# marqo-ai/marqo

Measured on NVIDIA H100. Metric: embeddings/s (open_clip/ViT-L-14 image vectorise, batch 256 per GPU), higher is better.
Workload: dtype bf16

## Files before the change

### marqo_b200/csrc/gemm.cu

```cuda
#include "gemm.cuh"

#include <mutex>
#include <type_traits>

#include "ptx.cuh"

namespace mb {
namespace gemm {

constexpr int BM = 128;
constexpr int BN = 128;
constexpr int BK = 64;
constexpr int WG_K = 16;
constexpr int STAGES = 3;
constexpr int MMA_THREADS = 256;
constexpr uint32_t A_STAGE_BYTES = BM * BK * 2;
constexpr uint32_t B_STAGE_BYTES = BN * BK * 2;
constexpr uint32_t STAGE_BYTES = A_STAGE_BYTES + B_STAGE_BYTES;
constexpr uint32_t BARRIER_BYTES = 256;
constexpr size_t SMEM_BYTES = (size_t)STAGES * STAGE_BYTES + 1024  + BARRIER_BYTES + 2 * BN * 4 ;
constexpr int EPI_ROWS = BM / 2;
constexpr uint32_t EPI_BOX_BYTES = EPI_ROWS * 128;
static_assert(4 * EPI_BOX_BYTES == STAGE_BYTES, "a warpgroup's fp32 64 x 128 block is one ring stage");

constexpr int P_BN = 256;
constexpr int P_STAGES = 3;
constexpr uint32_t P_STAGE_BYTES = A_STAGE_BYTES + P_BN * BK * 2;
constexpr uint32_t P_RING_BYTES = P_STAGES * P_STAGE_BYTES;
constexpr uint32_t EPI_BYTES = 4 * EPI_BOX_BYTES;
constexpr int PERSISTENT_THREADS = 128 + MMA_THREADS;
constexpr size_t P_SMEM_BYTES = 1024  + P_RING_BYTES + 2 * EPI_BYTES + 2 * P_BN * 4 + BARRIER_BYTES;
static_assert(P_SMEM_BYTES <= 227 * 1024, "over the opt-in shared memory of an H100 CTA");
static_assert(P_BN * 2 * EPI_ROWS == EPI_BYTES, "a warpgroup's bf16 64 x 256 block is one epilogue buffer");

enum Producer { PROD_TMA = 0, PROD_PATCH = 1, PROD_CONV = 2 };

template <bool GATHER>
constexpr int threads() { return MMA_THREADS + (GATHER ? 128 : 32); }

struct Params {
    int M, N, K;
    int tiles_m, tiles_n;
    Epilogue ep;
    const uint8_t* img;
    int g;
    int patch;
    int row_bytes;
    int seg;
    int kbpd;
    float nscale[3], nshift[3];
    int cls;
};

__device__ __forceinline__ float ex2_approx(float x) {
    float y;
    asm("ex2.approx.ftz.f32 %0, %1;" : "=f"(y) : "f"(x));
    return y;
}

__device__ __forceinline__ float gelu_erf(float x) {
    const float a = x * 0.70710678118654752440f;
    const float t = fabsf(a);
    const float s = a * a;
    float r = fmaf(-2.49374837e-5f, t, 5.52836593e-4f);
    const float u = fmaf(-5.60337594e-3f, t, 3.49920232e-2f);
    r = fmaf(r, s, u);
    r = fmaf(r, t, -1.54047912e-1f);
    r = fmaf(r, t, -9.15890168e-1f);
    r = fmaf(r, t, -1.85700115e-1f);
    r = fmaf(r, t, -1.44269504f * t);
    const float e = copysignf(1.0f - ex2_approx(r), a);
    const float hx = 0.5f * x;
    return fmaf(hx, e, hx);
}

__device__ __forceinline__ __half2 gelu_erf_h2(__half2 x) {
    const __half2 a = __hmul2(x, __float2half2_rn(0.70710678118654752440f));
    const __half2 t = __habs2(a);
    const __half2 s = __hmul2(a, a);
    __half2 r = __hfma2(__float2half2_rn(-2.49374837e-5f), t, __float2half2_rn(5.52836593e-4f));
    const __half2 u = __hfma2(__float2half2_rn(-5.60337594e-3f), t, __float2half2_rn(3.49920232e-2f));
    r = __hfma2(r, s, u);
    r = __hfma2(r, t, __float2half2_rn(-1.54047912e-1f));
    r = __hfma2(r, t, __float2half2_rn(-9.15890168e-1f));
    r = __hfma2(r, t, __float2half2_rn(-1.85700115e-1f));
    r = __hfma2(r, t, __hmul2(t, __float2half2_rn(-1.44269504f)));
    const __half2 e = h2exp2(r);
    const __half2 om = __hsub2(__float2half2_rn(1.0f), e);
    const uint32_t eb = (*reinterpret_cast<const uint32_t*>(&om) & 0x7fff7fffu) | (*reinterpret_cast<const uint32_t*>(&a) & 0x80008000u);
    const __half2 erfv = *reinterpret_cast<const __half2*>(&eb);
    const __half2 hx = __hmul2(x, __float2half2_rn(0.5f));
    return __hfma2(hx, erfv, hx);
}

__device__ __forceinline__ float quick_gelu(float x) {
    return x / (1.0f + ex2_approx(-1.702f * 1.44269504f * x));
}

__device__ __forceinline__ uint32_t sw128_offset(int row, int unit) {
    return (uint32_t)row * 128u + (uint32_t)((unit ^ (row & 7)) << 4);
}

template <int ELEM>
__device__ __forceinline__ uint32_t epi_offset(int row, int col) {
    constexpr int BOX_COLS = 128 / ELEM;
    const int byte = (col % BOX_COLS) * ELEM;
    return (uint32_t)(col / BOX_COLS) * EPI_BOX_BYTES + sw128_offset(row, byte >> 4) + (uint32_t)(byte & 15);
}

__device__ __forceinline__ void warpgroup_sync(int wg) {
    if (wg == 0)
        ptx::bar_sync<1, 128>();
    else
        ptx::bar_sync<2, 128>();
}

template <bool OUT_FP32, int ACT>
__device__ __forceinline__ float2 act(float x0, float x1) {
    if constexpr (ACT == ACT_GELU && !OUT_FP32) {
        float2 y = __half22float2(gelu_erf_h2(__floats2half2_rn(x0, x1)));
        y.x = x0 >= 65504.f ? x0 : x0 <= -65504.f ? -0.f : y.x;
        y.y = x1 >= 65504.f ? x1 : x1 <= -65504.f ? -0.f : y.y;
        return y;
    } else if constexpr (ACT == ACT_GELU)
        return make_float2(gelu_erf(x0), gelu_erf(x1));
    else if constexpr (ACT == ACT_QUICKGELU)
        return make_float2(quick_gelu(x0), quick_gelu(x1));
    else if constexpr (ACT == ACT_RELU)
        return make_float2(fmaxf(x0, 0.f), fmaxf(x1, 0.f));
    else
        return make_float2(x0, x1);
}

template <bool OUT_FP32, int ACT, int COLS>
__device__ __forceinline__ void epilogue_to_smem(const float* acc, uint32_t bias_s, uint32_t buf_s, bool residual,
                                                 int rbase, int lane) {
    static_assert(!(OUT_FP32 && ACT == ACT_RELU), "ACT_RELU writes bf16");
#pragma unroll
    for (int i = 0; i < COLS / 8; ++i) {
        const int col = 8 * i + 2 * (lane & 3);
        const float2 bv = ptx::ld_shared_f32x2(bias_s + 4 * col);
#pragma unroll
        for (int h = 0; h < 2; ++h) {
            const int r = rbase + 8 * h;
            if constexpr (ACT == ACT_RELU) {
                const uint32_t dst = buf_s + epi_offset<2>(r, col);
                float x0 = acc[4 * i + 2 * h] + bv.x, x1 = acc[4 * i + 2 * h + 1] + bv.y;
                if (residual) {
                    const uint32_t rv = ptx::ld_shared_u32(dst);
                    const float2 f = __bfloat1622float2(*reinterpret_cast<const __nv_bfloat162*>(&rv));
                    x0 += f.x;
                    x1 += f.y;
                }
                const float2 y = act<false, ACT_RELU>(x0, x1);
                ptx::st_shared_u32(dst, pack_bf16x2(y.x, y.y));
                continue;
            }
            float2 y = act<OUT_FP32, ACT>(acc[4 * i + 2 * h] + bv.x, acc[4 * i + 2 * h + 1] + bv.y);
            if constexpr (OUT_FP32) {
                const uint32_t dst = buf_s + epi_offset<4>(r, col);
                if (residual) {
                    const float2 rv = ptx::ld_shared_f32x2(dst);
                    y.x += rv.x;
                    y.y += rv.y;
                }
                ptx::st_shared_f32x2(dst, y.x, y.y);
            } else {
                ptx::st_shared_u32(buf_s + epi_offset<2>(r, col), pack_bf16x2(y.x, y.y));
            }
        }
    }
}

__device__ __forceinline__ void load_residual_boxes(const CUtensorMap* tmap_r, uint64_t* bar, uint8_t* buf, int row0,
                                                    int c0, int M, int N) {
    const int boxes = row0 < M && c0 < N ? min(4, (N - c0) / 32) : 0;
    ptx::mbar_arrive_expect_tx(bar, (uint32_t)boxes * EPI_BOX_BYTES);
    for (int b = 0; b < boxes; ++b)
        ptx::tma_load_2d(buf + b * EPI_BOX_BYTES, tmap_r, bar, c0 + 32 * b, row0, ptx::kEvictNormal);
}

__device__ __forceinline__ void load_residual_boxes_bf16(const CUtensorMap* tmap_r, uint64_t* bar, uint8_t* buf,
                                                         int row0, int c0, int M, int N) {
    const int boxes = row0 < M && c0 < N ? min(2, (N - c0 + 63) / 64) : 0;
    ptx::mbar_arrive_expect_tx(bar, (uint32_t)boxes * EPI_BOX_BYTES);
    for (int b = 0; b < boxes; ++b)
        ptx::tma_load_2d(buf + b * EPI_BOX_BYTES, tmap_r, bar, c0 + 64 * b, row0, ptx::kEvictNormal);
}

template <bool OUT_FP32, int COLS>
__device__ __forceinline__ void store_output_boxes(const CUtensorMap* tmap_o, const uint8_t* buf, int row0, int c0,
                                                   int M, int N) {
    constexpr int BOX_COLS = OUT_FP32 ? 32 : 64;
    if (row0 >= M) return;
    for (int b = 0; b * BOX_COLS < COLS && c0 + b * BOX_COLS < N; ++b)
        ptx::tma_store_2d(tmap_o, buf + b * EPI_BOX_BYTES, c0 + b * BOX_COLS, row0);
    ptx::tma_store_commit();
}

template <int PROD, bool OUT_FP32, int ACT>
__global__ void __launch_bounds__(threads<PROD != PROD_TMA>(), PROD != PROD_TMA ? 1 : 2)
gemm_kernel(const __grid_constant__ CUtensorMap tmap_a, const __grid_constant__ CUtensorMap tmap_b,
            const __grid_constant__ CUtensorMap tmap_r, const __grid_constant__ CUtensorMap tmap_o,
            const __grid_constant__ Params p) {
    constexpr bool GATHER = PROD != PROD_TMA;
    extern __shared__ uint8_t smem_raw[];
    uint8_t* smem = reinterpret_cast<uint8_t*>((reinterpret_cast<uintptr_t>(smem_raw) + 1023) & ~uintptr_t(1023));
    uint64_t* full = reinterpret_cast<uint64_t*>(smem + (size_t)STAGES * STAGE_BYTES);
    uint64_t* empty = full + STAGES;
    float* bias_s = reinterpret_cast<float*>(smem + (size_t)STAGES * STAGE_BYTES + BARRIER_BYTES);

    const int warp = __shfl_sync(0xffffffffu, threadIdx.x >> 5, 0);
    const int lane = threadIdx.x & 31;
    const int tile_m = blockIdx.x / p.tiles_n, tile_n = blockIdx.x % p.tiles_n;
    const int m0 = tile_m * BM, n0 = tile_n * BN;
    const int kblocks = p.K / BK;

    if (threadIdx.x == MMA_THREADS) {
        ptx::prefetch_tmap(&tmap_b);
        if (!GATHER) ptx::prefetch_tmap(&tmap_a);
        ptx::prefetch_tmap(&tmap_o);
        if (p.ep.residual) ptx::prefetch_tmap(&tmap_r);
        for (int i = 0; i < STAGES; ++i) {
            ptx::mbar_init(&full[i], GATHER ? 1 + 128 : 1);
            ptx::mbar_init(&empty[i], MMA_THREADS / 32);
        }
        ptx::fence_barrier_init();
    }
    __syncthreads();

    if (threadIdx.x >= MMA_THREADS) {
        const int pt = threadIdx.x - MMA_THREADS;
        if (!GATHER && pt >= 32) return;
        const uint8_t* prow = nullptr;
        const __nv_bfloat16* cimg = nullptr;
        int cy = 0, cx = 0;
        const int cH = p.g, cW = p.patch, lg_cin = p.kbpd;
        if (PROD == PROD_CONV) {
            const int r = m0 + pt;
            if (r < p.M) {
                const int hw = cH * cW;
                const int b = r / hw, rem = r - b * hw;
                cy = rem / cW;
                cx = rem - cy * cW;
                cimg = reinterpret_cast<const __nv_bfloat16*>(p.img) + ((size_t)b * hw << lg_cin);
            }
        }
        if (PROD == PROD_PATCH) {
            const int r = m0 + pt;
            const int tokens = p.g * p.g + p.cls;
            const int b = r / tokens, t = r - b * tokens - p.cls;
            if (r < p.M && t >= 0) {
                const int py = t / p.g, px = t - py * p.g;
                prow = p.img + ((size_t)b * p.g * p.patch + (size_t)py * p.patch) * p.row_bytes + (size_t)px * p.patch * 3;
            }
        }
        for (int kb = 0; kb < kblocks; ++kb) {
            const int stage = kb % STAGES;
            const uint32_t phase = (uint32_t)(kb / STAGES) & 1u;
            uint8_t* sa = smem + (size_t)stage * STAGE_BYTES;
            uint8_t* sb = sa + A_STAGE_BYTES;
            ptx::mbar_wait(&empty[stage], phase ^ 1);
            if (pt == 0) {
                ptx::mbar_arrive_expect_tx(&full[stage], GATHER ? B_STAGE_BYTES : STAGE_BYTES);
                if (!GATHER) ptx::tma_load_2d(sa, &tmap_a, &full[stage], kb * BK, m0, ptx::kEvictNormal);
                ptx::tma_load_2d(sb, &tmap_b, &full[stage], kb * BK, n0, ptx::kEvictLast);
            }
            if (PROD == PROD_CONV) {
                uint4 v[8];
#pragma unroll
                for (int u = 0; u < 8; ++u) {
                    const int k = kb * 64 + u * 8;
                    const int tap = k >> lg_cin, c = k & ((1 << lg_cin) - 1);
                    const int iy = cy + tap / 3 - 1, ix = cx + tap % 3 - 1;
                    v[u] = make_uint4(0u, 0u, 0u, 0u);
                    if (cimg != nullptr && tap < 9 && (unsigned)iy < (unsigned)cH && (unsigned)ix < (unsigned)cW)
                        v[u] = __ldg(reinterpret_cast<const uint4*>(cimg + (((size_t)iy * cW + ix) << lg_cin) + c));
                }
#pragma unroll
                for (int u = 0; u < 8; ++u) *reinterpret_cast<uint4*>(sa + sw128_offset(pt, u)) = v[u];
                ptx::fence_proxy_async_smem();
                ptx::mbar_arrive(&full[stage]);
            } else if (GATHER) {
                const int dy = kb / p.kbpd, j0 = (kb - dy * p.kbpd) * 64;
                const uint8_t* src = prow ? prow + (size_t)dy * p.row_bytes + j0 : nullptr;
                int c = j0 % 3;
#pragma unroll 1
                for (int u = 0; u < 8; ++u) {
                    uint32_t w[4];
#pragma unroll
                    for (int e = 0; e < 4; ++e) {
                        float v[2];
#pragma unroll
                        for (int h = 0; h < 2; ++h) {
                            const int j = u * 8 + e * 2 + h;
                            v[h] = (src != nullptr && j0 + j < p.seg) ? fmaf((float)__ldg(src + j), p.nscale[c], p.nshift[c]) : 0.f;
                            c = c == 2 ? 0 : c + 1;
                        }
                        w[e] = pack_bf16x2(v[0], v[1]);
                    }
                    *reinterpret_cast<uint4*>(sa + sw128_offset(pt, u)) = make_uint4(w[0], w[1], w[2], w[3]);
                }
                ptx::fence_proxy_async_smem();
                ptx::mbar_arrive(&full[stage]);
            }
        }
        for (int wg = 0; wg < 2; ++wg) {
            const int kb = kblocks + wg;
            const int stage = kb % STAGES;
            uint8_t* s = smem + (size_t)stage * STAGE_BYTES;
            ptx::mbar_wait(&empty[stage], ((uint32_t)(kb / STAGES) & 1u) ^ 1);
            if (pt == 0) {
                if (p.ep.residual != nullptr) {
                    if constexpr (ACT == ACT_RELU)
                        load_residual_boxes_bf16(&tmap_r, &full[stage], s, m0 + EPI_ROWS * wg, n0, p.M, p.N);
                    else
                        load_residual_boxes(&tmap_r, &full[stage], s, m0 + EPI_ROWS * wg, n0, p.M, p.N);
                } else
                    ptx::mbar_arrive(&full[stage]);
            }
            if (GATHER) ptx::mbar_arrive(&full[stage]);
        }
        return;
    }

    const int wg = warp >> 2;
    const Epilogue& ep = p.ep;
    float bias_t = 0.f;
    if (ep.bias != nullptr && n0 + (int)(threadIdx.x & 127) < p.N) bias_t = __ldg(ep.bias + n0 + (threadIdx.x & 127));
    float acc[BN / 2];
#pragma unroll
    for (int i = 0; i < BN / 2; ++i) acc[i] = 0.f;
    for (int kb = 0; kb < kblocks; ++kb) {
        const int stage = kb % STAGES;
        ptx::mbar_wait(&full[stage], (uint32_t)(kb / STAGES) & 1u);
        const uint32_t a_base = ptx::smem_u32(smem + (size_t)stage * STAGE_BYTES) + wg * (64 * 128);
        const uint32_t b_base = ptx::smem_u32(smem + (size_t)stage * STAGE_BYTES + A_STAGE_BYTES);
        ptx::wgmma_fence();
#pragma unroll
        for (int k = 0; k < BK / WG_K; ++k)
            ptx::wgmma_m64n128k16_bf16(acc, ptx::make_desc_k_sw128(a_base + k * WG_K * 2),
                                       ptx::make_desc_k_sw128(b_base + k * WG_K * 2), (kb | k) != 0 ? 1u : 0u);
        ptx::wgmma_commit();
        ptx::wgmma_wait<1>();
        if (kb > 0 && lane == 0) ptx::mbar_arrive(&empty[(kb - 1) % STAGES]);
    }
    ptx::wgmma_wait<0>();

    const int t = threadIdx.x & 127;
    float* wbias = bias_s + wg * BN;
    wbias[t] = bias_t;
    const int kb = kblocks + wg;
    ptx::mbar_wait(&full[kb % STAGES], (uint32_t)(kb / STAGES) & 1u);
    uint8_t* tile = smem + (size_t)(kb % STAGES) * STAGE_BYTES;
    warpgroup_sync(wg);
    const int rbase = (warp & 3) * 16 + (lane >> 2);
    epilogue_to_smem<OUT_FP32, ACT, BN>(acc, ptx::smem_u32(wbias), ptx::smem_u32(tile), ep.residual != nullptr, rbase,
                                        lane);
    ptx::fence_proxy_async_smem();
    warpgroup_sync(wg);
    if (t == 0) {
        store_output_boxes<OUT_FP32, BN>(&tmap_o, tile, m0 + EPI_ROWS * wg, n0, p.M, p.N);
        ptx::tma_store_wait_read<0>();
    }
}

template <bool OUT_FP32, int ACT>
__global__ void __launch_bounds__(PERSISTENT_THREADS, 1)
gemm_persistent_kernel(const __grid_constant__ CUtensorMap tmap_a, const __grid_constant__ CUtensorMap tmap_b,
                       const __grid_constant__ CUtensorMap tmap_r, const __grid_constant__ CUtensorMap tmap_o, Params p) {
    extern __shared__ uint8_t smem_raw[];
    uint8_t* smem = reinterpret_cast<uint8_t*>((reinterpret_cast<uintptr_t>(smem_raw) + 1023) & ~uintptr_t(1023));
    uint8_t* epi_s = smem + P_RING_BYTES;
    float* bias_s = reinterpret_cast<float*>(epi_s + 2 * EPI_BYTES);
    uint64_t* full = reinterpret_cast<uint64_t*>(bias_s + 2 * P_BN);
    uint64_t* empty = full + P_STAGES;
    uint64_t* epi_full = empty + P_STAGES;

    const int tiles = p.tiles_m * p.tiles_n;
    const int kblocks = p.K / BK;
    const Epilogue& ep = p.ep;
    const bool has_res = OUT_FP32 && ep.residual != nullptr;

    if (threadIdx.x == 0) {
        ptx::prefetch_tmap(&tmap_a);
        ptx::prefetch_tmap(&tmap_b);
        ptx::prefetch_tmap(&tmap_o);
        if (has_res) ptx::prefetch_tmap(&tmap_r);
        for (int i = 0; i < P_STAGES; ++i) {
            ptx::mbar_init(&full[i], 1);
            ptx::mbar_init(&empty[i], MMA_THREADS / 32);
        }
        ptx::mbar_init(&epi_full[0], 1);
        ptx::mbar_init(&epi_full[1], 1);
        ptx::fence_barrier_init();
    }
    __syncthreads();

    if (threadIdx.x < 128) {
        ptx::setmaxnreg_dec<40>();
        if (threadIdx.x != 0) return;
        uint32_t it = 0;
        for (int tile = blockIdx.x; tile < tiles; tile += gridDim.x) {
            const int m0 = (tile / p.tiles_n) * BM, n0 = (tile % p.tiles_n) * P_BN;
            for (int kb = 0; kb < kblocks; ++kb, ++it) {
                const int stage = it % P_STAGES;
                uint8_t* sa = smem + (size_t)stage * P_STAGE_BYTES;
                ptx::mbar_wait(&empty[stage], ((it / P_STAGES) & 1u) ^ 1);
                ptx::mbar_arrive_expect_tx(&full[stage], P_STAGE_BYTES);
                ptx::tma_load_2d(sa, &tmap_a, &full[stage], kb * BK, m0, ptx::kEvictNormal);
                ptx::tma_load_2d(sa + A_STAGE_BYTES, &tmap_b, &full[stage], kb * BK, n0, ptx::kEvictLast);
            }
        }
        return;
    }

    ptx::setmaxnreg_inc<232>();
    const int wg = (threadIdx.x >> 7) - 1;
    const int t = threadIdx.x & 127;
    const int warp = t >> 5, lane = t & 31;
    uint8_t* buf = epi_s + wg * EPI_BYTES;
    float* wbias = bias_s + wg * P_BN;
    const uint32_t buf_s = ptx::smem_u32(buf), wbias_s = ptx::smem_u32(wbias);
    const int rbase = warp * 16 + (lane >> 2);
    constexpr int COLS = OUT_FP32 ? 128 : P_BN;
    uint32_t it = 0, epi_phase = 0;

    for (int tile = blockIdx.x; tile < tiles; tile += gridDim.x) {
        const int m0 = (tile / p.tiles_n) * BM, n0 = (tile % p.tiles_n) * P_BN;
        const int row0 = m0 + EPI_ROWS * wg;
        float bias_r[P_BN / 128];
#pragma unroll
        for (int j = 0; j < P_BN / 128; ++j) {
            const int c = n0 + t + 128 * j;
            bias_r[j] = ep.bias != nullptr && c < p.N ? __ldg(ep.bias + c) : 0.f;
        }
        float acc[P_BN / 2];
#pragma unroll
        for (int i = 0; i < P_BN / 2; ++i) acc[i] = 0.f;
        for (int kb = 0; kb < kblocks; ++kb, ++it) {
            const int stage = it % P_STAGES;
            ptx::mbar_wait(&full[stage], (it / P_STAGES) & 1u);
            const uint32_t a_base = ptx::smem_u32(smem + (size_t)stage * P_STAGE_BYTES) + wg * (64 * 128);
            const uint32_t b_base = ptx::smem_u32(smem + (size_t)stage * P_STAGE_BYTES + A_STAGE_BYTES);
            ptx::wgmma_fence();
#pragma unroll
            for (int k = 0; k < BK / WG_K; ++k) {
                const uint64_t da = ptx::make_desc_k_sw128(a_base + k * WG_K * 2);
                const uint64_t db = ptx::make_desc_k_sw128(b_base + k * WG_K * 2);
                ptx::wgmma_m64n256k16_bf16(acc, da, db, (kb | k) != 0 ? 1u : 0u);
            }
            ptx::wgmma_commit();
            ptx::wgmma_wait<1>();
            if (kb > 0 && lane == 0) ptx::mbar_arrive(&empty[(it - 1) % P_STAGES]);
            if (kb == 0 && t == 0) {
                ptx::tma_store_wait_read<0>();
                if (has_res) {
                    load_residual_boxes(&tmap_r, &epi_full[wg], buf, row0, n0, p.M, p.N);
                    if (row0 < p.M)
                        for (int b = 0; b < 4 && n0 + 128 + 32 * b < p.N; ++b)
                            ptx::tma_prefetch_l2_2d(&tmap_r, n0 + 128 + 32 * b, row0);
                }
            }
        }
        ptx::wgmma_wait<0>();
        if (lane == 0) ptx::mbar_arrive(&empty[(it - 1) % P_STAGES]);

#pragma unroll
        for (int j = 0; j < P_BN / 128; ++j) wbias[t + 128 * j] = bias_r[j];
        warpgroup_sync(wg);
#pragma unroll
        for (int hf = 0; hf < P_BN / COLS; ++hf) {
            if (hf > 0) {
                if (t == 0) {
                    ptx::tma_store_wait_read<0>();
                    if (has_res) load_residual_boxes(&tmap_r, &epi_full[wg], buf, row0, n0 + COLS * hf, p.M, p.N);
                }
                if (!has_res) warpgroup_sync(wg);
            }
            if (has_res) {
                ptx::mbar_wait(&epi_full[wg], epi_phase);
                epi_phase ^= 1;
            }
            epilogue_to_smem<OUT_FP32, ACT, COLS>(acc + COLS / 2 * hf, wbias_s + 4 * COLS * hf, buf_s, has_res, rbase,
                                                  lane);
            ptx::fence_proxy_async_smem();
            warpgroup_sync(wg);
            if (t == 0) store_output_boxes<OUT_FP32, COLS>(&tmap_o, buf, row0, n0 + COLS * hf, p.M, p.N);
        }
    }
    if (t == 0) ptx::tma_store_wait_read<0>();
}

template <class F>
static void dispatch(bool out_fp32, int act, F&& f) {
    if (act == ACT_RELU) {
        f(std::false_type{}, std::integral_constant<int, ACT_RELU>{});
        return;
    }
    const auto with_act = [&](auto out) {
        if (act == ACT_GELU)
            f(out, std::integral_constant<int, ACT_GELU>{});
        else if (act == ACT_QUICKGELU)
            f(out, std::integral_constant<int, ACT_QUICKGELU>{});
        else
            f(out, std::integral_constant<int, ACT_NONE>{});
    };
    if (out_fp32)
        with_act(std::true_type{});
    else
        with_act(std::false_type{});
}

void configure() {
    static std::once_flag once;
    std::call_once(once, [] {
        const auto attr = cudaFuncAttributeMaxDynamicSharedMemorySize;
        MB_CUDA(cudaFuncSetAttribute(gemm_kernel<PROD_PATCH, true, ACT_NONE>, attr, (int)SMEM_BYTES));
        MB_CUDA(cudaFuncSetAttribute(gemm_kernel<PROD_CONV, false, ACT_RELU>, attr, (int)SMEM_BYTES));
        for (int out_fp32 = 0; out_fp32 < 2; ++out_fp32)
            for (int act = ACT_NONE; act <= ACT_RELU; ++act)
                dispatch(out_fp32, act, [&](auto out, auto a) {
                    constexpr bool OUT_FP32 = decltype(out)::value;
                    constexpr int ACT = decltype(a)::value;
                    MB_CUDA(cudaFuncSetAttribute(gemm_kernel<PROD_TMA, OUT_FP32, ACT>, attr, (int)SMEM_BYTES));
                    MB_CUDA(cudaFuncSetAttribute(gemm_persistent_kernel<OUT_FP32, ACT>, attr, (int)P_SMEM_BYTES));
                });
    });
}

static void check_epilogue(const Epilogue& ep) {
    if (ep.ldo % 8 != 0) fail(B200_ERR_INTERNAL, "gemm: ldo = %d must be a multiple of 8", ep.ldo);
    if ((reinterpret_cast<uintptr_t>(ep.out) & 15) != 0) fail(B200_ERR_INTERNAL, "gemm: output not 16-byte aligned");
    if (ep.act == ACT_RELU && ep.out_fp32) fail(B200_ERR_INTERNAL, "gemm: ReLU writes a bf16 output");
    if (ep.residual != nullptr && (ep.out_fp32 ? ep.ldr % 4 != 0 : ep.act != ACT_RELU || ep.ldr % 8 != 0))
        fail(B200_ERR_INTERNAL, "gemm: the residual needs an fp32 output and ldr %% 4 == 0, or ReLU and ldr %% 8 == 0");
    if (ep.residual != nullptr && (reinterpret_cast<uintptr_t>(ep.residual) & 15) != 0)
        fail(B200_ERR_INTERNAL, "gemm: residual not 16-byte aligned");
}

static void epilogue_tmaps(const Epilogue& ep, int M, int N, CUtensorMap& tr, CUtensorMap& to) {
    if (ep.residual)
        tr = ep.out_fp32 ? make_tmap_2d(ep.residual, CU_TENSOR_MAP_DATA_TYPE_FLOAT32, 4, (uint64_t)N, (uint64_t)M,
                                        (uint64_t)ep.ldr * 4, 32, EPI_ROWS, CU_TENSOR_MAP_SWIZZLE_128B)
                         : make_tmap_2d(ep.residual, CU_TENSOR_MAP_DATA_TYPE_BFLOAT16, 2, (uint64_t)N, (uint64_t)M,
                                        (uint64_t)ep.ldr * 2, 64, EPI_ROWS, CU_TENSOR_MAP_SWIZZLE_128B);
    to = ep.out_fp32 ? make_tmap_2d(ep.out, CU_TENSOR_MAP_DATA_TYPE_FLOAT32, 4, (uint64_t)N, (uint64_t)M,
                                    (uint64_t)ep.ldo * 4, 32, EPI_ROWS, CU_TENSOR_MAP_SWIZZLE_128B)
                     : make_tmap_2d(ep.out, CU_TENSOR_MAP_DATA_TYPE_BFLOAT16, 2, (uint64_t)N, (uint64_t)M,
                                    (uint64_t)ep.ldo * 2, 64, EPI_ROWS, CU_TENSOR_MAP_SWIZZLE_128B);
}

template <int PROD, bool OUT_FP32, int ACT>
static void launch_tiles(const __nv_bfloat16* A, int lda, const __nv_bfloat16* W, int M, int N, int K, const Epilogue& ep,
                         cudaStream_t stream, const PatchGather* pg = nullptr, const ConvGather* cg = nullptr) {
    constexpr bool GATHER = PROD != PROD_TMA;
    Params p{};
    if (PROD == PROD_CONV) {
        p.img = reinterpret_cast<const uint8_t*>(cg->act);
        p.g = cg->H;
        p.patch = cg->W;
        while ((1 << p.kbpd) < cg->cin) ++p.kbpd;
    }
    if (PROD == PROD_PATCH) {
        p.img = pg->img;
        p.patch = pg->patch;
        p.g = pg->S / pg->patch;
        p.row_bytes = 3 * pg->S;
        p.seg = 3 * pg->patch;
        p.kbpd = patch_gather_kbpd(pg->patch);
        p.cls = pg->cls;
        for (int c = 0; c < 3; ++c) {
            p.nscale[c] = (float)(1.0 / (255.0 * (double)pg->std[c]));
            p.nshift[c] = (float)(-(double)pg->mean[c] / (double)pg->std[c]);
        }
    }
    p.M = M;
    p.N = N;
    p.K = K;
    p.tiles_n = (N + BN - 1) / BN;
    p.ep = ep;
    const long long tiles = (long long)((M + BM - 1) / BM) * p.tiles_n;
    if (tiles > 0x7fffffffLL) fail(B200_ERR_UNSUPPORTED, "gemm: %lld tiles is too many", tiles);
    CUtensorMap tb = make_tmap_2d(W, CU_TENSOR_MAP_DATA_TYPE_BFLOAT16, 2, (uint64_t)K, (uint64_t)N, (uint64_t)K * 2, BK, BN,
                                  CU_TENSOR_MAP_SWIZZLE_128B);
    CUtensorMap ta = GATHER ? tb
                            : make_tmap_2d(A, CU_TENSOR_MAP_DATA_TYPE_BFLOAT16, 2, (uint64_t)K, (uint64_t)M,
                                           (uint64_t)lda * 2, BK, BM, CU_TENSOR_MAP_SWIZZLE_128B);
    CUtensorMap tr = tb, to;
    epilogue_tmaps(ep, M, N, tr, to);
    gemm_kernel<PROD, OUT_FP32, ACT><<<(unsigned)tiles, threads<GATHER>(), SMEM_BYTES, stream>>>(ta, tb, tr, to, p);
    MB_CUDA(cudaGetLastError());
}

template <bool OUT_FP32, int ACT>
static void launch_persistent(const __nv_bfloat16* A, int lda, const __nv_bfloat16* W, int M, int N, int K,
                              const Epilogue& ep, int sms, cudaStream_t stream) {
    Params p{};
    p.M = M;
    p.N = N;
    p.K = K;
    p.tiles_m = (M + BM - 1) / BM;
    p.tiles_n = (N + P_BN - 1) / P_BN;
    p.ep = ep;
    const long long tiles = (long long)p.tiles_m * p.tiles_n;
    if (tiles > 0x7fffffffLL) fail(B200_ERR_UNSUPPORTED, "gemm: %lld tiles is too many", tiles);
    CUtensorMap ta = make_tmap_2d(A, CU_TENSOR_MAP_DATA_TYPE_BFLOAT16, 2, (uint64_t)K, (uint64_t)M, (uint64_t)lda * 2,
                                  BK, BM, CU_TENSOR_MAP_SWIZZLE_128B);
    CUtensorMap tb = make_tmap_2d(W, CU_TENSOR_MAP_DATA_TYPE_BFLOAT16, 2, (uint64_t)K, (uint64_t)N, (uint64_t)K * 2, BK,
                                  P_BN, CU_TENSOR_MAP_SWIZZLE_128B);
    CUtensorMap tr = tb, to;
    epilogue_tmaps(ep, M, N, tr, to);
    const int grid = (int)std::min<long long>(tiles, std::max(sms, 1));
    gemm_persistent_kernel<OUT_FP32, ACT><<<grid, PERSISTENT_THREADS, P_SMEM_BYTES, stream>>>(ta, tb, tr, to, p);
    MB_CUDA(cudaGetLastError());
}

int launch_patch_embed(const PatchGather& pg, const __nv_bfloat16* Wg, int N, const Epilogue& ep, cudaStream_t stream) {
    if (pg.n <= 0 || N <= 0) return 0;
    if (pg.S <= 0 || pg.patch <= 0 || pg.S % pg.patch != 0)
        fail(B200_ERR_INTERNAL, "patch gather: image %d is not a multiple of patch %d", pg.S, pg.patch);
    if (N % 32 != 0) fail(B200_ERR_INTERNAL, "patch gather: N = %d must be a multiple of 32", N);
    if (!ep.out_fp32 || ep.act != ACT_NONE) fail(B200_ERR_INTERNAL, "patch gather: fp32 output without activation only");
    check_epilogue(ep);
    configure();
    if (pg.cls != 0 && pg.cls != 1) fail(B200_ERR_INTERNAL, "patch gather: cls = %d must be 0 or 1", pg.cls);
    const int g = pg.S / pg.patch;
    const long long M = (long long)pg.n * (g * g + pg.cls);
    if (M > 0x7fffffffLL) fail(B200_ERR_INVALID_ARG, "patch gather: batch of %d images is too large", pg.n);
    launch_tiles<PROD_PATCH, true, ACT_NONE>(nullptr, 0, Wg, (int)M, N, patch_gather_k(pg.patch), ep, stream, &pg);
    return 1;
}

int launch_conv3x3(const ConvGather& cg, const __nv_bfloat16* Wc, int N, const Epilogue& ep, cudaStream_t stream) {
    if (cg.n <= 0 || N <= 0) return 0;
    if (cg.H <= 0 || cg.W <= 0 || cg.cin < 32 || (cg.cin & (cg.cin - 1)) != 0)
        fail(B200_ERR_INTERNAL, "conv3x3: %d x %d x %d input (cin must be a power of two >= 32)", cg.H, cg.W, cg.cin);
    if (N % 32 != 0) fail(B200_ERR_INTERNAL, "conv3x3: N = %d must be a multiple of 32", N);
    if (ep.out_fp32 || ep.act != ACT_RELU) fail(B200_ERR_INTERNAL, "conv3x3: bf16 output with ReLU only");
    if ((reinterpret_cast<uintptr_t>(cg.act) & 15) != 0) fail(B200_ERR_INTERNAL, "conv3x3: input not 16-byte aligned");
    check_epilogue(ep);
    configure();
    const long long M = (long long)cg.n * cg.H * cg.W;
    if (M > 0x7fffffffLL) fail(B200_ERR_INVALID_ARG, "conv3x3: batch of %d images is too large", cg.n);
// ... 57 lines not shown
```

### marqo_b200/csrc/ptx.cuh

```cuda
#pragma once
#include <cstdint>
#include <cstdio>
#include <cuda.h>
#include <cuda_runtime.h>

namespace ptx {

__device__ __forceinline__ uint32_t smem_u32(const void* p) {
    return static_cast<uint32_t>(__cvta_generic_to_shared(p));
}

__device__ __forceinline__ void st_shared_u32(uint32_t addr, uint32_t v) {
    asm volatile("st.shared.b32 [%0], %1;" ::"r"(addr), "r"(v) : "memory");
}
__device__ __forceinline__ void st_shared_f32x2(uint32_t addr, float x, float y) {
    asm volatile("st.shared.v2.f32 [%0], {%1, %2};" ::"r"(addr), "f"(x), "f"(y) : "memory");
}
__device__ __forceinline__ uint32_t ld_shared_u32(uint32_t addr) {
    uint32_t v;
    asm volatile("ld.shared.b32 %0, [%1];" : "=r"(v) : "r"(addr) : "memory");
    return v;
}
__device__ __forceinline__ float2 ld_shared_f32x2(uint32_t addr) {
    float2 v;
    asm volatile("ld.shared.v2.f32 {%0, %1}, [%2];" : "=f"(v.x), "=f"(v.y) : "r"(addr) : "memory");
    return v;
}

__device__ __forceinline__ uint32_t lane_id() {
    uint32_t l;
    asm volatile("mov.u32 %0, %%laneid;" : "=r"(l));
    return l;
}

__device__ __forceinline__ uint64_t globaltimer_ns() {
    uint64_t t;
    asm volatile("mov.u64 %0, %%globaltimer;" : "=l"(t));
    return t;
}

__device__ __forceinline__ bool elect_one() {
    uint32_t pred;
    asm volatile(
        "{\n"
        ".reg .pred p;\n"
        "elect.sync _|p, 0xffffffff;\n"
        "selp.u32 %0, 1, 0, p;\n"
        "}\n"
        : "=r"(pred));
    return pred != 0;
}

__device__ __forceinline__ void mbar_init(uint64_t* bar, uint32_t count) {
    asm volatile("mbarrier.init.shared::cta.b64 [%0], %1;" ::"r"(smem_u32(bar)), "r"(count) : "memory");
}
__device__ __forceinline__ void fence_barrier_init() {
    asm volatile("fence.mbarrier_init.release.cluster;" ::: "memory");
}
__device__ __forceinline__ void fence_proxy_async_smem() {
    asm volatile("fence.proxy.async.shared::cta;" ::: "memory");
}
__device__ __forceinline__ void mbar_arrive_expect_tx(uint64_t* bar, uint32_t bytes) {
    asm volatile("mbarrier.arrive.expect_tx.shared::cta.b64 _, [%0], %1;" ::"r"(smem_u32(bar)), "r"(bytes)
                 : "memory");
}
__device__ __forceinline__ void mbar_arrive(uint64_t* bar) {
    asm volatile("mbarrier.arrive.shared::cta.b64 _, [%0];" ::"r"(smem_u32(bar)) : "memory");
}
__device__ __forceinline__ bool mbar_try_wait(uint64_t* bar, uint32_t parity) {
    uint32_t ok;
    asm volatile(
        "{\n"
        ".reg .pred p;\n"
        "mbarrier.try_wait.parity.shared::cta.b64 p, [%1], %2;\n"
        "selp.u32 %0, 1, 0, p;\n"
        "}\n"
        : "=r"(ok)
        : "r"(smem_u32(bar)), "r"(parity)
        : "memory");
    return ok != 0;
}
__device__ __forceinline__ void mbar_wait(uint64_t* bar, uint32_t parity) {
    if (mbar_try_wait(bar, parity)) return;
    uint64_t t0 = globaltimer_ns();
    uint32_t spins = 0;
    while (!mbar_try_wait(bar, parity)) {
        if ((++spins & 0x3ff) == 0 && globaltimer_ns() - t0 > 4000000000ull) __trap();
    }
}

constexpr uint64_t kEvictNormal = 0x1000000000000000ull;
constexpr uint64_t kEvictFirst = 0x12F0000000000000ull;
constexpr uint64_t kEvictLast = 0x14F0000000000000ull;

__device__ __forceinline__ void prefetch_tmap(const CUtensorMap* tmap) {
    asm volatile("prefetch.tensormap [%0];" ::"l"(reinterpret_cast<uint64_t>(tmap)) : "memory");
}

__device__ __forceinline__ void tma_load_2d(void* smem_dst, const CUtensorMap* tmap, uint64_t* bar, int32_t c0,
                                            int32_t c1, uint64_t cache_hint) {
    asm volatile(
        "cp.async.bulk.tensor.2d.shared::cluster.global.tile.mbarrier::complete_tx::bytes.L2::cache_hint"
        " [%0], [%1, {%3, %4}], [%2], %5;"
        ::"r"(smem_u32(smem_dst)), "l"(reinterpret_cast<uint64_t>(tmap)), "r"(smem_u32(bar)), "r"(c0), "r"(c1),
        "l"(cache_hint)
        : "memory");
}

__device__ __forceinline__ void tma_prefetch_l2_2d(const CUtensorMap* tmap, int32_t c0, int32_t c1) {
    asm volatile("cp.async.bulk.prefetch.tensor.2d.L2.global.tile [%0, {%1, %2}];" ::"l"(reinterpret_cast<uint64_t>(tmap)),
                 "r"(c0), "r"(c1)
                 : "memory");
}

__device__ __forceinline__ void tma_store_2d(const CUtensorMap* tmap, const void* smem_src, int32_t c0, int32_t c1) {
    asm volatile("cp.async.bulk.tensor.2d.global.shared::cta.tile.bulk_group [%0, {%2, %3}], [%1];" ::"l"(
                     reinterpret_cast<uint64_t>(tmap)),
                 "r"(smem_u32(smem_src)), "r"(c0), "r"(c1)
                 : "memory");
}
__device__ __forceinline__ void tma_store_commit() { asm volatile("cp.async.bulk.commit_group;" ::: "memory"); }
template <int N>
__device__ __forceinline__ void tma_store_wait_read() {
    asm volatile("cp.async.bulk.wait_group.read %0;" ::"n"(N) : "memory");
}
template <int N>
__device__ __forceinline__ void tma_store_wait() {
    asm volatile("cp.async.bulk.wait_group %0;" ::"n"(N) : "memory");
}

__device__ __forceinline__ uint64_t make_desc_k_sw128(uint32_t smem_addr) {
    uint64_t d = 0;
    d |= static_cast<uint64_t>((smem_addr & 0x3FFFF) >> 4);
    d |= static_cast<uint64_t>(1) << 16;
    d |= static_cast<uint64_t>(1024 >> 4) << 32;
    d |= static_cast<uint64_t>(1) << 62;
    return d;
}

__device__ __forceinline__ uint64_t make_desc_mn_sw128(uint32_t smem_addr, uint32_t lbo_bytes) {
    uint64_t d = 0;
    d |= static_cast<uint64_t>((smem_addr & 0x3FFFF) >> 4);
    d |= static_cast<uint64_t>((lbo_bytes >> 4) & 0x3FFF) << 16;
    d |= static_cast<uint64_t>(1024 >> 4) << 32;
    d |= static_cast<uint64_t>(1) << 62;
    return d;
}

__device__ __forceinline__ uint64_t make_desc_k_sw64(uint32_t smem_addr) {
    uint64_t d = 0;
    d |= static_cast<uint64_t>((smem_addr & 0x3FFFF) >> 4);
    d |= static_cast<uint64_t>(1) << 16;
    d |= static_cast<uint64_t>(512 >> 4) << 32;
    d |= static_cast<uint64_t>(2) << 62;
    return d;
}

__device__ __forceinline__ uint64_t make_desc_mn_sw64(uint32_t smem_addr, uint32_t lbo_bytes) {
    uint64_t d = 0;
    d |= static_cast<uint64_t>((smem_addr & 0x3FFFF) >> 4);
    d |= static_cast<uint64_t>((lbo_bytes >> 4) & 0x3FFF) << 16;
    d |= static_cast<uint64_t>(512 >> 4) << 32;
    d |= static_cast<uint64_t>(2) << 62;
    return d;
}

__device__ __forceinline__ void wgmma_fence() { asm volatile("wgmma.fence.sync.aligned;" ::: "memory"); }
__device__ __forceinline__ void wgmma_commit() { asm volatile("wgmma.commit_group.sync.aligned;" ::: "memory"); }
template <int N>
__device__ __forceinline__ void wgmma_wait() {
    asm volatile("wgmma.wait_group.sync.aligned %0;" ::"n"(N) : "memory");
}

__device__ __forceinline__ void wgmma_m64n128k16_f16(float (&d)[64], uint64_t desc_a, uint64_t desc_b, uint32_t scale_d) {
    asm volatile(
        "{\n"
        ".reg .pred p;\n"
        "setp.ne.b32 p, %66, 0;\n"
        "wgmma.mma_async.sync.aligned.m64n128k16.f32.f16.f16 "
        "{"
        "%0, %1, %2, %3, %4, %5, %6, %7, %8, %9, %10, %11, %12, %13, %14, %15, "
        "%16, %17, %18, %19, %20, %21, %22, %23, %24, %25, %26, %27, %28, %29, %30, %31, "
        "%32, %33, %34, %35, %36, %37, %38, %39, %40, %41, %42, %43, %44, %45, %46, %47, "
        "%48, %49, %50, %51, %52, %53, %54, %55, %56, %57, %58, %59, %60, %61, %62, %63"
        "}, %64, %65, p, 1, 1, 0, 0;\n"
        "}\n"
        : "+f"(d[0]), "+f"(d[1]), "+f"(d[2]), "+f"(d[3]), "+f"(d[4]), "+f"(d[5]), "+f"(d[6]), "+f"(d[7]),
          "+f"(d[8]), "+f"(d[9]), "+f"(d[10]), "+f"(d[11]), "+f"(d[12]), "+f"(d[13]), "+f"(d[14]), "+f"(d[15]),
          "+f"(d[16]), "+f"(d[17]), "+f"(d[18]), "+f"(d[19]), "+f"(d[20]), "+f"(d[21]), "+f"(d[22]), "+f"(d[23]),
          "+f"(d[24]), "+f"(d[25]), "+f"(d[26]), "+f"(d[27]), "+f"(d[28]), "+f"(d[29]), "+f"(d[30]), "+f"(d[31]),
          "+f"(d[32]), "+f"(d[33]), "+f"(d[34]), "+f"(d[35]), "+f"(d[36]), "+f"(d[37]), "+f"(d[38]), "+f"(d[39]),
          "+f"(d[40]), "+f"(d[41]), "+f"(d[42]), "+f"(d[43]), "+f"(d[44]), "+f"(d[45]), "+f"(d[46]), "+f"(d[47]),
          "+f"(d[48]), "+f"(d[49]), "+f"(d[50]), "+f"(d[51]), "+f"(d[52]), "+f"(d[53]), "+f"(d[54]), "+f"(d[55]),
          "+f"(d[56]), "+f"(d[57]), "+f"(d[58]), "+f"(d[59]), "+f"(d[60]), "+f"(d[61]), "+f"(d[62]), "+f"(d[63])
        : "l"(desc_a), "l"(desc_b), "r"(scale_d));
}
__device__ __forceinline__ void wgmma_m64n128k16_bf16(float (&d)[64], uint64_t desc_a, uint64_t desc_b, uint32_t scale_d) {
    asm volatile(
        "{\n"
        ".reg .pred p;\n"
        "setp.ne.b32 p, %66, 0;\n"
        "wgmma.mma_async.sync.aligned.m64n128k16.f32.bf16.bf16 "
        "{"
        "%0, %1, %2, %3, %4, %5, %6, %7, %8, %9, %10, %11, %12, %13, %14, %15, "
        "%16, %17, %18, %19, %20, %21, %22, %23, %24, %25, %26, %27, %28, %29, %30, %31, "
        "%32, %33, %34, %35, %36, %37, %38, %39, %40, %41, %42, %43, %44, %45, %46, %47, "
        "%48, %49, %50, %51, %52, %53, %54, %55, %56, %57, %58, %59, %60, %61, %62, %63"
        "}, %64, %65, p, 1, 1, 0, 0;\n"
        "}\n"
        : "+f"(d[0]), "+f"(d[1]), "+f"(d[2]), "+f"(d[3]), "+f"(d[4]), "+f"(d[5]), "+f"(d[6]), "+f"(d[7]),
          "+f"(d[8]), "+f"(d[9]), "+f"(d[10]), "+f"(d[11]), "+f"(d[12]), "+f"(d[13]), "+f"(d[14]), "+f"(d[15]),
          "+f"(d[16]), "+f"(d[17]), "+f"(d[18]), "+f"(d[19]), "+f"(d[20]), "+f"(d[21]), "+f"(d[22]), "+f"(d[23]),
          "+f"(d[24]), "+f"(d[25]), "+f"(d[26]), "+f"(d[27]), "+f"(d[28]), "+f"(d[29]), "+f"(d[30]), "+f"(d[31]),
          "+f"(d[32]), "+f"(d[33]), "+f"(d[34]), "+f"(d[35]), "+f"(d[36]), "+f"(d[37]), "+f"(d[38]), "+f"(d[39]),
          "+f"(d[40]), "+f"(d[41]), "+f"(d[42]), "+f"(d[43]), "+f"(d[44]), "+f"(d[45]), "+f"(d[46]), "+f"(d[47]),
          "+f"(d[48]), "+f"(d[49]), "+f"(d[50]), "+f"(d[51]), "+f"(d[52]), "+f"(d[53]), "+f"(d[54]), "+f"(d[55]),
          "+f"(d[56]), "+f"(d[57]), "+f"(d[58]), "+f"(d[59]), "+f"(d[60]), "+f"(d[61]), "+f"(d[62]), "+f"(d[63])
        : "l"(desc_a), "l"(desc_b), "r"(scale_d));
}
__device__ __forceinline__ void wgmma_m64n256k16_bf16(float (&d)[128], uint64_t desc_a, uint64_t desc_b, uint32_t scale_d) {
    asm volatile(
        "{\n"
        ".reg .pred p;\n"
        "setp.ne.b32 p, %130, 0;\n"
        "wgmma.mma_async.sync.aligned.m64n256k16.f32.bf16.bf16 "
        "{"
        "%0, %1, %2, %3, %4, %5, %6, %7, %8, %9, %10, %11, %12, %13, %14, %15, "
        "%16, %17, %18, %19, %20, %21, %22, %23, %24, %25, %26, %27, %28, %29, %30, %31, "
        "%32, %33, %34, %35, %36, %37, %38, %39, %40, %41, %42, %43, %44, %45, %46, %47, "
        "%48, %49, %50, %51, %52, %53, %54, %55, %56, %57, %58, %59, %60, %61, %62, %63, "
        "%64, %65, %66, %67, %68, %69, %70, %71, %72, %73, %74, %75, %76, %77, %78, %79, "
        "%80, %81, %82, %83, %84, %85, %86, %87, %88, %89, %90, %91, %92, %93, %94, %95, "
        "%96, %97, %98, %99, %100, %101, %102, %103, %104, %105, %106, %107, %108, %109, %110, %111, "
        "%112, %113, %114, %115, %116, %117, %118, %119, %120, %121, %122, %123, %124, %125, %126, %127"
        "}, %128, %129, p, 1, 1, 0, 0;\n"
        "}\n"
        : "+f"(d[0]), "+f"(d[1]), "+f"(d[2]), "+f"(d[3]), "+f"(d[4]), "+f"(d[5]), "+f"(d[6]), "+f"(d[7]),
          "+f"(d[8]), "+f"(d[9]), "+f"(d[10]), "+f"(d[11]), "+f"(d[12]), "+f"(d[13]), "+f"(d[14]), "+f"(d[15]),
          "+f"(d[16]), "+f"(d[17]), "+f"(d[18]), "+f"(d[19]), "+f"(d[20]), "+f"(d[21]), "+f"(d[22]), "+f"(d[23]),
          "+f"(d[24]), "+f"(d[25]), "+f"(d[26]), "+f"(d[27]), "+f"(d[28]), "+f"(d[29]), "+f"(d[30]), "+f"(d[31]),
          "+f"(d[32]), "+f"(d[33]), "+f"(d[34]), "+f"(d[35]), "+f"(d[36]), "+f"(d[37]), "+f"(d[38]), "+f"(d[39]),
          "+f"(d[40]), "+f"(d[41]), "+f"(d[42]), "+f"(d[43]), "+f"(d[44]), "+f"(d[45]), "+f"(d[46]), "+f"(d[47]),
          "+f"(d[48]), "+f"(d[49]), "+f"(d[50]), "+f"(d[51]), "+f"(d[52]), "+f"(d[53]), "+f"(d[54]), "+f"(d[55]),
          "+f"(d[56]), "+f"(d[57]), "+f"(d[58]), "+f"(d[59]), "+f"(d[60]), "+f"(d[61]), "+f"(d[62]), "+f"(d[63]),
          "+f"(d[64]), "+f"(d[65]), "+f"(d[66]), "+f"(d[67]), "+f"(d[68]), "+f"(d[69]), "+f"(d[70]), "+f"(d[71]),
          "+f"(d[72]), "+f"(d[73]), "+f"(d[74]), "+f"(d[75]), "+f"(d[76]), "+f"(d[77]), "+f"(d[78]), "+f"(d[79]),
          "+f"(d[80]), "+f"(d[81]), "+f"(d[82]), "+f"(d[83]), "+f"(d[84]), "+f"(d[85]), "+f"(d[86]), "+f"(d[87]),
          "+f"(d[88]), "+f"(d[89]), "+f"(d[90]), "+f"(d[91]), "+f"(d[92]), "+f"(d[93]), "+f"(d[94]), "+f"(d[95]),
          "+f"(d[96]), "+f"(d[97]), "+f"(d[98]), "+f"(d[99]), "+f"(d[100]), "+f"(d[101]), "+f"(d[102]), "+f"(d[103]),
          "+f"(d[104]), "+f"(d[105]), "+f"(d[106]), "+f"(d[107]), "+f"(d[108]), "+f"(d[109]), "+f"(d[110]), "+f"(d[111]),
          "+f"(d[112]), "+f"(d[113]), "+f"(d[114]), "+f"(d[115]), "+f"(d[116]), "+f"(d[117]), "+f"(d[118]), "+f"(d[119]),
          "+f"(d[120]), "+f"(d[121]), "+f"(d[122]), "+f"(d[123]), "+f"(d[124]), "+f"(d[125]), "+f"(d[126]), "+f"(d[127])
        : "l"(desc_a), "l"(desc_b), "r"(scale_d));
}
__device__ __forceinline__ void wgmma_m64n64k16_bf16_rs_tb(float (&d)[32], const uint32_t (&a)[4], uint64_t desc_b, uint32_t scale_d) {
    asm volatile(
        "{\n"
        ".reg .pred p;\n"
        "setp.ne.b32 p, %37, 0;\n"
        "wgmma.mma_async.sync.aligned.m64n64k16.f32.bf16.bf16 "
        "{"
        "%0, %1, %2, %3, %4, %5, %6, %7, %8, %9, %10, %11, %12, %13, %14, %15, "
        "%16, %17, %18, %19, %20, %21, %22, %23, %24, %25, %26, %27, %28, %29, %30, %31"
        "}, {%32, %33, %34, %35}, %36, p, 1, 1, 1;\n"
        "}\n"
        : "+f"(d[0]), "+f"(d[1]), "+f"(d[2]), "+f"(d[3]), "+f"(d[4]), "+f"(d[5]), "+f"(d[6]), "+f"(d[7]),
          "+f"(d[8]), "+f"(d[9]), "+f"(d[10]), "+f"(d[11]), "+f"(d[12]), "+f"(d[13]), "+f"(d[14]), "+f"(d[15]),
          "+f"(d[16]), "+f"(d[17]), "+f"(d[18]), "+f"(d[19]), "+f"(d[20]), "+f"(d[21]), "+f"(d[22]), "+f"(d[23]),
          "+f"(d[24]), "+f"(d[25]), "+f"(d[26]), "+f"(d[27]), "+f"(d[28]), "+f"(d[29]), "+f"(d[30]), "+f"(d[31])
        : "r"(a[0]), "r"(a[1]), "r"(a[2]), "r"(a[3]), "l"(desc_b), "r"(scale_d));
}
__device__ __forceinline__ void wgmma_m64n32k16_bf16_rs_tb(float (&d)[16], const uint32_t (&a)[4], uint64_t desc_b, uint32_t scale_d) {
    asm volatile(
        "{\n"
        ".reg .pred p;\n"
        "setp.ne.b32 p, %21, 0;\n"
        "wgmma.mma_async.sync.aligned.m64n32k16.f32.bf16.bf16 "
        "{"
        "%0, %1, %2, %3, %4, %5, %6, %7, %8, %9, %10, %11, %12, %13, %14, %15"
        "}, {%16, %17, %18, %19}, %20, p, 1, 1, 1;\n"
        "}\n"
        : "+f"(d[0]), "+f"(d[1]), "+f"(d[2]), "+f"(d[3]), "+f"(d[4]), "+f"(d[5]), "+f"(d[6]), "+f"(d[7]),
          "+f"(d[8]), "+f"(d[9]), "+f"(d[10]), "+f"(d[11]), "+f"(d[12]), "+f"(d[13]), "+f"(d[14]), "+f"(d[15])
        : "r"(a[0]), "r"(a[1]), "r"(a[2]), "r"(a[3]), "l"(desc_b), "r"(scale_d));
}
template <int REGS>
__device__ __forceinline__ void setmaxnreg_inc() {
    asm volatile("setmaxnreg.inc.sync.aligned.u32 %0;" ::"n"(REGS));
}
template <int REGS>
__device__ __forceinline__ void setmaxnreg_dec() {
    asm volatile("setmaxnreg.dec.sync.aligned.u32 %0;" ::"n"(REGS));
}

template <int ID, int COUNT>
__device__ __forceinline__ void bar_sync() {
    asm volatile("bar.sync %0, %1;" ::"n"(ID), "n"(COUNT) : "memory");
}

}
```

Before: 2757.

## Offload bf16 GELU and output stores to idle producer warps in persistent GEMM

For the bf16 GELU persistent GEMM, the MMA warpgroups now write only bias-added fp16-rounded pre-activations to shared memory. Three otherwise idle producer-warpgroup warps then apply the fp16 GELU polynomial in place, convert to bf16 and issue the TMA stores, handing buffers back through new staged/drained mbarriers. This lets the MMA warps start the next tile's wgmma sooner instead of running the transcendental epilogue themselves. A warpgroup-wide OR reduction detects values at or beyond the fp16 range and falls back to the old in-warp epilogue for that tile. Register budgets shift from MMA to producer warps, which may add spill pressure, and the residual path is disabled under this mode.

```diff
diff --git a/marqo_b200/csrc/gemm.cu b/marqo_b200/csrc/gemm.cu
--- a/marqo_b200/csrc/gemm.cu
+++ b/marqo_b200/csrc/gemm.cu
@@ -32,6 +32,7 @@
 constexpr size_t P_SMEM_BYTES = 1024  + P_RING_BYTES + 2 * EPI_BYTES + 2 * P_BN * 4 + BARRIER_BYTES;
 static_assert(P_SMEM_BYTES <= 227 * 1024, "over the opt-in shared memory of an H100 CTA");
 static_assert(P_BN * 2 * EPI_ROWS == EPI_BYTES, "a warpgroup's bf16 64 x 256 block is one epilogue buffer");
+static_assert((2 * P_STAGES + 3 * 2) * 8 + 2 * 4 <= BARRIER_BYTES, "the persistent kernel's mbarriers and flags");
 
 enum Producer { PROD_TMA = 0, PROD_PATCH = 1, PROD_CONV = 2 };
 
@@ -93,6 +94,19 @@
     return __hfma2(hx, erfv, hx);
 }
 
+__device__ __forceinline__ uint32_t gelu_h2_round(float x0, float x1) {
+    const __half2 h = __floats2half2_rn(x0, x1);
+    return *reinterpret_cast<const uint32_t*>(&h);
+}
+__device__ __forceinline__ float2 gelu_h2_eval(uint32_t h) {
+    return __half22float2(gelu_erf_h2(*reinterpret_cast<const __half2*>(&h)));
+}
+__device__ __forceinline__ uint32_t gelu_h2_bf16(uint32_t h) {
+    const float2 y = gelu_h2_eval(h);
+    return pack_bf16x2(y.x, y.y);
+}
+constexpr float FP16_EDGE = 65504.f;
+
 __device__ __forceinline__ float quick_gelu(float x) {
     return x / (1.0f + ex2_approx(-1.702f * 1.44269504f * x));
 }
@@ -114,13 +128,17 @@
     else
         ptx::bar_sync<2, 128>();
 }
+__device__ __forceinline__ bool warpgroup_any(int wg, bool pred) {
+    return wg == 0 ? ptx::bar_red_or<1, 128>(pred) : ptx::bar_red_or<2, 128>(pred);
+}
+__device__ __forceinline__ void epilogue_warps_sync() { ptx::bar_sync<3, 96>(); }
 
 template <bool OUT_FP32, int ACT>
 __device__ __forceinline__ float2 act(float x0, float x1) {
     if constexpr (ACT == ACT_GELU && !OUT_FP32) {
-        float2 y = __half22float2(gelu_erf_h2(__floats2half2_rn(x0, x1)));
-        y.x = x0 >= 65504.f ? x0 : x0 <= -65504.f ? -0.f : y.x;
-        y.y = x1 >= 65504.f ? x1 : x1 <= -65504.f ? -0.f : y.y;
+        float2 y = gelu_h2_eval(gelu_h2_round(x0, x1));
+        y.x = x0 >= FP16_EDGE ? x0 : x0 <= -FP16_EDGE ? -0.f : y.x;
+        y.y = x1 >= FP16_EDGE ? x1 : x1 <= -FP16_EDGE ? -0.f : y.y;
         return y;
     } else if constexpr (ACT == ACT_GELU)
         return make_float2(gelu_erf(x0), gelu_erf(x1));
@@ -132,10 +150,12 @@
         return make_float2(x0, x1);
 }
 
-template <bool OUT_FP32, int ACT, int COLS>
-__device__ __forceinline__ void epilogue_to_smem(const float* acc, uint32_t bias_s, uint32_t buf_s, bool residual,
+template <bool OUT_FP32, int ACT, int COLS, bool GELU_ROUND = false>
+__device__ __forceinline__ bool epilogue_to_smem(const float* acc, uint32_t bias_s, uint32_t buf_s, bool residual,
                                                  int rbase, int lane) {
     static_assert(!(OUT_FP32 && ACT == ACT_RELU), "ACT_RELU writes bf16");
+    static_assert(!GELU_ROUND || (!OUT_FP32 && ACT == ACT_GELU), "GELU_ROUND is the bf16 GELU's first half");
+    float xmax[2] = {0.f, 0.f};
 #pragma unroll
     for (int i = 0; i < COLS / 8; ++i) {
         const int col = 8 * i + 2 * (lane & 3);
@@ -156,6 +176,12 @@
                 ptx::st_shared_u32(dst, pack_bf16x2(y.x, y.y));
                 continue;
             }
+            if constexpr (GELU_ROUND) {
+                const float x0 = acc[4 * i + 2 * h] + bv.x, x1 = acc[4 * i + 2 * h + 1] + bv.y;
+                xmax[h] = fmaxf(xmax[h], fmaxf(fabsf(x0), fabsf(x1)));
+                ptx::st_shared_u32(buf_s + epi_offset<2>(r, col), gelu_h2_round(x0, x1));
+                continue;
+            }
             float2 y = act<OUT_FP32, ACT>(acc[4 * i + 2 * h] + bv.x, acc[4 * i + 2 * h + 1] + bv.y);
             if constexpr (OUT_FP32) {
                 const uint32_t dst = buf_s + epi_offset<4>(r, col);
@@ -170,6 +196,7 @@
             }
         }
     }
+    return fmaxf(xmax[0], xmax[1]) >= FP16_EDGE;
 }
 
 __device__ __forceinline__ void load_residual_boxes(const CUtensorMap* tmap_r, uint64_t* bar, uint8_t* buf, int row0,
@@ -376,6 +403,9 @@
     uint64_t* full = reinterpret_cast<uint64_t*>(bias_s + 2 * P_BN);
     uint64_t* empty = full + P_STAGES;
     uint64_t* epi_full = empty + P_STAGES;
+    uint64_t* staged = epi_full + 2;
+    uint64_t* drained = staged + 2;
+    const uint32_t gelu_wide_s = ptx::smem_u32(drained + 2);
 
     const int tiles = p.tiles_m * p.tiles_n;
     const int kblocks = p.K / BK;
@@ -391,31 +421,72 @@
             ptx::mbar_init(&full[i], 1);
             ptx::mbar_init(&empty[i], MMA_THREADS / 32);
         }
-        ptx::mbar_init(&epi_full[0], 1);
-        ptx::mbar_init(&epi_full[1], 1);
+        for (int i = 0; i < 2; ++i) {
+            ptx::mbar_init(&epi_full[i], 1);
+            ptx::mbar_init(&staged[i], 4);
+            ptx::mbar_init(&drained[i], 1);
+        }
         ptx::fence_barrier_init();
     }
     __syncthreads();
 
+    constexpr bool EPI_WARPS = !OUT_FP32 && ACT == ACT_GELU;
+    constexpr int PRODUCER_REGS = EPI_WARPS ? 56 : 40, MMA_REGS = EPI_WARPS ? 224 : 232;
+    static_assert(128 * PRODUCER_REGS + MMA_THREADS * MMA_REGS == PERSISTENT_THREADS * 168, "the CTA's registers");
     if (threadIdx.x < 128) {
-        ptx::setmaxnreg_dec<40>();
-        if (threadIdx.x != 0) return;
-        uint32_t it = 0;
-        for (int tile = blockIdx.x; tile < tiles; tile += gridDim.x) {
-            const int m0 = (tile / p.tiles_n) * BM, n0 = (tile % p.tiles_n) * P_BN;
-            for (int kb = 0; kb < kblocks; ++kb, ++it) {
-                const int stage = it % P_STAGES;
-                uint8_t* sa = smem + (size_t)stage * P_STAGE_BYTES;
-                ptx::mbar_wait(&empty[stage], ((it / P_STAGES) & 1u) ^ 1);
-                ptx::mbar_arrive_expect_tx(&full[stage], P_STAGE_BYTES);
-                ptx::tma_load_2d(sa, &tmap_a, &full[stage], kb * BK, m0, ptx::kEvictNormal);
-                ptx::tma_load_2d(sa + A_STAGE_BYTES, &tmap_b, &full[stage], kb * BK, n0, ptx::kEvictLast);
+        ptx::setmaxnreg_dec<PRODUCER_REGS>();
+        if (threadIdx.x == 0) {
+            uint32_t it = 0;
+            for (int tile = blockIdx.x; tile < tiles; tile += gridDim.x) {
+                const int m0 = (tile / p.tiles_n) * BM, n0 = (tile % p.tiles_n) * P_BN;
+                for (int kb = 0; kb < kblocks; ++kb, ++it) {
+                    const int stage = it % P_STAGES;
+                    uint8_t* sa = smem + (size_t)stage * P_STAGE_BYTES;
+                    ptx::mbar_wait(&empty[stage], ((it / P_STAGES) & 1u) ^ 1);
+                    ptx::mbar_arrive_expect_tx(&full[stage], P_STAGE_BYTES);
+                    ptx::tma_load_2d(sa, &tmap_a, &full[stage], kb * BK, m0, ptx::kEvictNormal);
+                    ptx::tma_load_2d(sa + A_STAGE_BYTES, &tmap_b, &full[stage], kb * BK, n0, ptx::kEvictLast);
+                }
+            }
+        } else if (EPI_WARPS && threadIdx.x >= 32) {
+            const uint32_t et = threadIdx.x - 32;
+            uint32_t phase = 0;
+            for (int tile = blockIdx.x; tile < tiles; tile += gridDim.x, phase ^= 1) {
+                const int m0 = (tile / p.tiles_n) * BM, n0 = (tile % p.tiles_n) * P_BN;
+                for (int wg = 0; wg < 2; ++wg) {
+                    uint8_t* buf = epi_s + wg * EPI_BYTES;
+                    ptx::mbar_wait(&staged[wg], phase);
+                    if (ptx::ld_shared_u32(gelu_wide_s + 4 * wg) == 0) {
+                        const uint32_t buf_s = ptx::smem_u32(buf);
+                        for (uint32_t u = et; u < EPI_BYTES / 16; u += 2 * 96) {
+                            const bool second = u + 96 < EPI_BYTES / 16;
+                            uint4 v[2] = {ptx::ld_shared_u32x4(buf_s + 16 * u), make_uint4(0u, 0u, 0u, 0u)};
+                            if (second) v[1] = ptx::ld_shared_u32x4(buf_s + 16 * (u + 96));
+#pragma unroll
+                            for (int j = 0; j < 2; ++j) {
+                                v[j].x = gelu_h2_bf16(v[j].x);
+                                v[j].y = gelu_h2_bf16(v[j].y);
+                                v[j].z = gelu_h2_bf16(v[j].z);
+                                v[j].w = gelu_h2_bf16(v[j].w);
+                            }
+                            ptx::st_shared_u32x4(buf_s + 16 * u, v[0]);
+                            if (second) ptx::st_shared_u32x4(buf_s + 16 * (u + 96), v[1]);
+                        }
+                        ptx::fence_proxy_async_smem();
+                    }
+                    epilogue_warps_sync();
+                    if (et == 0) {
+                        store_output_boxes<false, P_BN>(&tmap_o, buf, m0 + EPI_ROWS * wg, n0, p.M, p.N);
+                        ptx::tma_store_wait_read<0>();
+                        ptx::mbar_arrive(&drained[wg]);
+                    }
+                }
             }
         }
         return;
     }
 
-    ptx::setmaxnreg_inc<232>();
+    ptx::setmaxnreg_inc<MMA_REGS>();
     const int wg = (threadIdx.x >> 7) - 1;
     const int t = threadIdx.x & 127;
     const int warp = t >> 5, lane = t & 31;
@@ -423,10 +494,9 @@
     float* wbias = bias_s + wg * P_BN;
     const uint32_t buf_s = ptx::smem_u32(buf), wbias_s = ptx::smem_u32(wbias);
     const int rbase = warp * 16 + (lane >> 2);
-    constexpr int COLS = OUT_FP32 ? 128 : P_BN;
-    uint32_t it = 0, epi_phase = 0;
-
-    for (int tile = blockIdx.x; tile < tiles; tile += gridDim.x) {
+    uint32_t it = 0, epi_phase = 0, phase = 0;
+
+    for (int tile = blockIdx.x; tile < tiles; tile += gridDim.x, phase ^= 1) {
         const int m0 = (tile / p.tiles_n) * BM, n0 = (tile % p.tiles_n) * P_BN;
         const int row0 = m0 + EPI_ROWS * wg;
         float bias_r[P_BN / 128];
@@ -453,7 +523,7 @@
             ptx::wgmma_commit();
             ptx::wgmma_wait<1>();
             if (kb > 0 && lane == 0) ptx::mbar_arrive(&empty[(it - 1) % P_STAGES]);
-            if (kb == 0 && t == 0) {
+            if (!EPI_WARPS && kb == 0 && t == 0) {
                 ptx::tma_store_wait_read<0>();
                 if (has_res) {
                     load_residual_boxes(&tmap_r, &epi_full[wg], buf, row0, n0, p.M, p.N);
@@ -466,6 +536,22 @@
         ptx::wgmma_wait<0>();
         if (lane == 0) ptx::mbar_arrive(&empty[(it - 1) % P_STAGES]);
 
+        if constexpr (EPI_WARPS) {
+            ptx::mbar_wait(&drained[wg], phase ^ 1);
+#pragma unroll
+            for (int j = 0; j < P_BN / 128; ++j) wbias[t + 128 * j] = bias_r[j];
+            warpgroup_sync(wg);
+            const bool wide = warpgroup_any(
+                wg, epilogue_to_smem<false, ACT_GELU, P_BN, true>(acc, wbias_s, buf_s, false, rbase, lane));
+            if (t == 0) ptx::st_shared_u32(gelu_wide_s + 4 * wg, wide ? 1u : 0u);
+            if (wide) epilogue_to_smem<false, ACT_GELU, P_BN>(acc, wbias_s, buf_s, false, rbase, lane);
+            ptx::fence_proxy_async_smem();
+            __syncwarp();
+            if (lane == 0) ptx::mbar_arrive(&staged[wg]);
+            continue;
+        }
+
+        constexpr int COLS = OUT_FP32 ? 128 : P_BN;
 #pragma unroll
         for (int j = 0; j < P_BN / 128; ++j) wbias[t + 128 * j] = bias_r[j];
         warpgroup_sync(wg);
@@ -489,7 +575,7 @@
             if (t == 0) store_output_boxes<OUT_FP32, COLS>(&tmap_o, buf, row0, n0 + COLS * hf, p.M, p.N);
         }
     }
-    if (t == 0) ptx::tma_store_wait_read<0>();
+    if (!EPI_WARPS && t == 0) ptx::tma_store_wait_read<0>();
 }
 
 template <class F>
diff --git a/marqo_b200/csrc/ptx.cuh b/marqo_b200/csrc/ptx.cuh
--- a/marqo_b200/csrc/ptx.cuh
+++ b/marqo_b200/csrc/ptx.cuh
@@ -25,6 +25,16 @@
     float2 v;
     asm volatile("ld.shared.v2.f32 {%0, %1}, [%2];" : "=f"(v.x), "=f"(v.y) : "r"(addr) : "memory");
     return v;
+}
+__device__ __forceinline__ uint4 ld_shared_u32x4(uint32_t addr) {
+    uint4 v;
+    asm volatile("ld.shared.v4.b32 {%0, %1, %2, %3}, [%4];" : "=r"(v.x), "=r"(v.y), "=r"(v.z), "=r"(v.w) : "r"(addr)
+                 : "memory");
+    return v;
+}
+__device__ __forceinline__ void st_shared_u32x4(uint32_t addr, uint4 v) {
+    asm volatile("st.shared.v4.b32 [%0], {%1, %2, %3, %4};" ::"r"(addr), "r"(v.x), "r"(v.y), "r"(v.z), "r"(v.w)
+                 : "memory");
 }
 
 __device__ __forceinline__ uint32_t lane_id() {
@@ -297,5 +307,20 @@
 __device__ __forceinline__ void bar_sync() {
     asm volatile("bar.sync %0, %1;" ::"n"(ID), "n"(COUNT) : "memory");
 }
-
-}
+template <int ID, int COUNT>
+__device__ __forceinline__ bool bar_red_or(bool pred) {
+    uint32_t any;
+    asm volatile(
+        "{\n"
+        ".reg .pred p, q;\n"
+        "setp.ne.u32 p, %1, 0;\n"
+        "bar.red.or.pred q, %2, %3, p;\n"
+        "selp.u32 %0, 1, 0, q;\n"
+        "}\n"
+        : "=r"(any)
+        : "r"((uint32_t)pred), "n"(ID), "n"(COUNT)
+        : "memory");
+    return any != 0;
+}
+
+}
```

New measurement: 2796 (median of 6 runs). 1.4% higher.
